# RHnejad/3D_PoseEstimation

Measured on AMD Instinct MI355X. Metric: poses/sec fwd+bwd, 17-joint lifting batch 4096; MPJPE vs ref, higher is better.
Workload: dtype f16x3 (two fp16 planes per fp32 operand, 3 fp16 MFMAs per product, fp32 accumulate); 1 GPU; BASELINE configs[1]: phase1_lifting LinearModel 34-1024-2x(1024-1024)-51, BN+ReLU+Dropout(0.5), one train_1.py step = zero_grad+forward+MSE+backward+AdamW; launch=hipgraph (one hipGraph replay per step), per_gpu_batch=4096, global_batch=4096, parallelism=dp1

## Files before the change

3d_poseestimation_amd/csrc/api.hip:

```cpp
#include <stdarg.h>
#include <stdio.h>
#include <stdlib.h>

#include <vector>

#include "adamw.h"
#include "pl_internal.h"

namespace pl {

static thread_local char g_err[512] = "";

void set_error(const char* fmt, ...) {
  va_list ap;
  va_start(ap, fmt);
  vsnprintf(g_err, sizeof(g_err), fmt, ap);
  va_end(ap);
}

namespace {

inline int64_t align_up(int64_t v, int64_t a) { return (v + a - 1) / a * a; }

int check_desc(const PLDesc* d, bool need_arenas) {
// ... 75 lines not shown

int out_splits(int M, int N, int K) {
  const int tiles = ((M + 127) / 128) * ((N + 127) / 128);
  int s = 256 / tiles;
  const int kmax = K / 128;
  if (s > kmax) s = kmax;
  return s < 1 ? 1 : s;
}

enum class Lin : uint8_t {
  Skinny, Planes, Gemm,
  PlanesMid,
  F32Mid,
};
enum class Stats : uint8_t {
  None,
  InLayer,
  Small,
  InApply,
  Finalize,
};
enum class Bwd : uint8_t {
  PlanesPair, F32Pair,
  SmallLayer, SmallLayerDw,
  InAbove,
  First,
};
struct LayerRoute {
  Lin lin;
  Stats stats;
  Bwd bwd;
  int groups;
  bool bnr_fused;
};
enum class Loss : uint8_t { SmallMse, FromSlabs, PartialOnly };

struct Ws {
  int L, G, RC;
  std::vector<size_t> z, act, bits, mean, rstd, dbpart;
  size_t stat, scale, shift, coef, ga, gb, dz, slabs, outpart, dyout, mse, total;
  size_t act_bytes, bits_bytes;
  size_t slab_floats;
  bool planes;
  int pkind;
  std::vector<size_t> actp, wp;
  std::vector<size_t> sactp;
  std::vector<char> act_f32;
  size_t dzp, amax, dzscale;
  size_t skp_out, skp_in;
  std::vector<size_t> wslab;
  std::vector<LayerRoute> layer;
  bool bn_small;
  bool small_layer;
  bool top_fused;
  bool adam_rides;
  bool small_f16;
  bool eval_small;
  bool out_narrow;
  bool out_skinny;
  Loss loss;
};

Ws plan(const PLDesc* d, int64_t B) {
  Ws w;
  w.L = 1 + 2 * d->num_stage;
  const int H = d->hidden;
  w.G = gemm_stat_groups((int)B);
  w.RC = bwd_row_chunks((int)B, H);
  size_t o = 0;
  auto take = [&](size_t bytes) {
    const size_t at = o;
    o = (size_t)align_up((int64_t)(o + bytes), 256);
    return at;
// ... 25 lines not shown
  auto need = [&](int M, int N) {
    const int s = tn_splits(M, N, (int)B);
    if (s > 1) slab = std::max(slab, (size_t)s * M * N * 4);
  };
  need(H, d->in_dim);
  need(H, H);
  need(d->out_dim, H);
  {
    const int so = out_splits((int)B, d->out_dim, H);
    if (so > 1) slab = std::max(slab, (size_t)so * B * d->out_dim * 4);
    slab = std::max(slab, (size_t)skinny_chunks((int)B) * std::max(d->in_dim, d->out_dim) * H * 4);
    slab = std::max(slab, skinny_narrow_out_part_floats((int)B, H) * 4);
    if (B <= kThinGemmMaxM && B % 128) slab = std::max(slab, thin_gemm_scratch_floats((int)B, H, H) * 4);
    if (B <= kThinGemmMaxM) slab = std::max(slab, (size_t)(H / 16 + 1) * B * 64 * 4);
  }
  w.slab_floats = slab / 4;
  w.slabs = take(slab);
  w.outpart = take((size_t)std::max(colsum_chunks((int)B), skinny_in_chunks((int)B)) * d->out_dim * 4);
  w.dyout = take((size_t)B * d->out_dim * 4);
  w.mse = take(std::max(pl_mse_scratch_bytes(B * d->out_dim), (size_t)256));
  w.dzp = w.amax = w.dzscale = 0;
  w.skp_out = take((size_t)skinny_in_chunks((int)B) * d->out_dim * H * 4);
  w.skp_in = take((size_t)skinny_in_chunks((int)B) * d->in_dim * H * 4);
  if (w.planes) {
    w.wslab.push_back(0);
    for (int l = 1; l < w.L; ++l) w.wslab.push_back(take((size_t)tn_splits(H, H, (int)B) * H * H * 4));
    for (int l = 0; l + 1 < w.L; ++l) w.actp.push_back(take(w.act_bytes));
    w.wp.push_back(0);
    for (int l = 1; l < w.L; ++l) w.wp.push_back(take((size_t)H * H * 4));
    w.dzp = take(w.act_bytes);
    w.amax = take(std::max((size_t)((H + 255) / 256) * w.RC, (size_t)(B / 64) * (H / 32)) * 2 * 4);
    w.dzscale = take((size_t)w.L * 2 * 4);
  }
  if (d->dtype == PL_F16X3 && B <= kThinGemmMaxM)
    for (int l = 0; l + 1 < w.L; ++l) w.sactp.push_back(take(w.act_bytes));
  w.total = o;

  const int world = sync_world(d);
  const bool first_ok = small_first_ok(d->in_dim), mid_ok = B * world <= 512 && small_layer_ok(2, H, H);
  w.bn_small = d->bn && !w.planes && world == 1 && B >= 2 && B <= kBnSmallRows;
  w.small_layer = w.bn_small && small_layer_ok((int)B, H, H);
  w.top_fused = w.small_layer && small_top_ok(d->out_dim);
  const bool small_head = w.top_fused && (d->num_stage > 0 || first_ok);
  w.adam_rides = small_head && H % 128 == 0;
  w.small_f16 = d->dtype == PL_F16X3 && !w.sactp.empty() && first_ok;
  w.eval_small = d->bn && B <= kThinGemmMaxM && small_layer_ok(2, H, H) && first_ok && small_top_ok(d->out_dim);
  w.out_narrow = skinny_narrow_out_supported(H, d->out_dim);
  w.out_skinny = skinny_supported(d->out_dim, H);
  const int so = w.out_narrow ? skinny_narrow_out_splits((int)B, H) : 0;
  w.loss = small_head ? Loss::SmallMse : (so && mse_from_slabs_supported(so, d->out_dim)) ? Loss::FromSlabs : Loss::PartialOnly;
  for (int l = 0; l < w.L; ++l) {
    LayerRoute r;
    if (l == 0) r.lin = skinny_supported(d->in_dim, H) ? Lin::Skinny : Lin::Gemm;
    else if (w.planes) r.lin = w.pkind == 2 && mid_ok ? Lin::PlanesMid : Lin::Planes;
    else r.lin = d->bn && d->dtype != PL_BF16 && B > kBnSmallRows && mid_ok ? Lin::F32Mid : Lin::Gemm;
    r.groups = r.lin == Lin::Skinny ? skinny_stat_groups((int)B) : w.G;
    const bool tile = w.small_layer && (l > 0 || first_ok);
    if (!d->bn) r.stats = Stats::None;
    else if (w.bn_small) r.stats = tile ? Stats::InLayer : Stats::Small;
    else r.stats = world == 1 && r.groups >= 1 && r.groups <= 4 ? Stats::InApply : Stats::Finalize;
    if (l == 0) r.bwd = tile && w.L > 1 ? Bwd::InAbove : Bwd::First;
    else if (!w.small_layer) r.bwd = w.planes ? Bwd::PlanesPair : Bwd::F32Pair;
    else r.bwd = H % 128 == 0 ? Bwd::SmallLayerDw : Bwd::SmallLayer;
    r.bnr_fused = w.planes && (l < w.L - 1 || w.out_skinny);
    w.layer.push_back(r);
  }
  return w;
}

struct BnrSlab {
  float *mine, *amax_mine, *amax0;
  int64_t floats_per_rank;
  int world;
};
BnrSlab bnr_slab(const PLDesc* d, const Ws& w, void* ws, int rc, int n_amax, bool eval_bn) {
  BnrSlab b;
  float* stat = reinterpret_cast<float*>(static_cast<char*>(ws) + w.stat);
  b.world = eval_bn ? 1 : sync_world(d);
  const int64_t sums = (int64_t)2 * rc * d->hidden;
  if (b.world == 1) {
    b.mine = stat;
    b.amax_mine = b.amax0 = w.amax ? reinterpret_cast<float*>(static_cast<char*>(ws) + w.amax) : nullptr;
    b.floats_per_rank = sums;
    return b;
  }
// ... 159 lines not shown
}

extern "C" size_t pl_workspace_bytes(const PLDesc* d, int64_t B) {
  if (check_desc(d, false) != PL_OK || B <= 0) return 0;
  return plan(d, B).total;
}

extern "C" int pl_workspace_view(const PLDesc* d, int64_t B, int which, int64_t layer, size_t* off,
                                 size_t* size) {
  PL_TRY(check_desc(d, false));
  if (B <= 0 || !off || !size) PL_FAIL(PL_EINVAL, "pl_workspace_view: bad arguments");
  const Ws w = plan(d, B);
  if (layer < 0 || layer >= w.L) PL_FAIL(PL_EINVAL, "pl_workspace_view: layer %lld out of range", (long long)layer);
  const size_t hb = (size_t)d->hidden * 4;
  switch (which) {
    case 0: *off = w.z[layer]; *size = w.act_bytes; break;
    case 1:
      if (!w.act_f32[layer])
        PL_FAIL(PL_EINVAL, "pl_workspace_view: the planes path keeps the output of hidden layer %lld as 16-bit planes only", (long long)layer);
      *off = w.act[layer]; *size = w.act_bytes; break;
    case 2: *off = w.bits[layer]; *size = w.bits_bytes; break;
    case 3: *off = w.mean[layer]; *size = hb; break;
    case 4: *off = w.rstd[layer]; *size = hb; break;
    default: PL_FAIL(PL_EINVAL, "pl_workspace_view: which=%d", which);
  }
  return PL_OK;
}

extern "C" int pl_workspace_bitmap_format(const PLDesc* d, int64_t B, int64_t layer) {
  PL_TRY(check_desc(d, false));
  if (B <= 0 || layer < 0 || layer >= 1 + 2 * (int64_t)d->num_stage) PL_FAIL(PL_EINVAL, "pl_workspace_bitmap_format: bad arguments");
  return plan(d, B).layer[layer].stats == Stats::InLayer ? 1 : 0;
}

extern "C" int pl_lifter_fwd_eval(const PLDesc* d, const float* x, float* y, int64_t B, void* ws,
                                  size_t ws_bytes, void* stream) {
  PL_TRY(check_desc(d, true));
  if (!x || !y) PL_FAIL(PL_EINVAL, "pl_lifter_fwd_eval: null x/y");
  if (B <= 0) PL_FAIL(PL_ESHAPE, "pl_lifter_fwd_eval: B=%lld", (long long)B);
  const Ws w = plan(d, B);
  PL_TRY(check_ws(w, ws, ws_bytes));
  const ParamLayout P = param_layout(d);
  hipStream_t s = (hipStream_t)stream;
  const int H = d->hidden;
  if (w.eval_small) {
    const float* a_in = x;
// ... 211 lines not shown
                                 false, f32(ws, w.outpart)));
    job(f32(ws, w.skp_out), grads + P.off[4 * w.L], skinny_in_chunks(Bi), O * H, 0, 0);
    job(f32(ws, w.outpart), grads + P.off[4 * w.L + 1], skinny_in_chunks(Bi), O, 0, 0);
    GemmArgs be = {};
    const int lt = w.L - 1;
    if (!eval_bn && w.layer[lt].bnr_fused) {
      const BnrSlab sl = bnr_slab(d, w, ws, Bi / 64, (w.pkind == 2 && lt > 0) ? (Bi / 64) * (H / 32) : 0, eval_bn);
      be.bnr_z = f32(ws, w.z[lt]); be.bnr_bits = u64(ws, w.bits[lt]);
      be.bnr_mean = f32(ws, w.mean[lt]); be.bnr_rstd = f32(ws, w.rstd[lt]); be.bnr_kscale = kscale;
      be.bnr_part_dy = sl.mine; be.bnr_part_dyz = sl.mine + (size_t)(Bi / 64) * H;
      be.bnr_amax = (w.pkind == 2 && lt > 0) ? sl.amax_mine : nullptr;
    }
    PL_TRY(launch_skinny_wide_out(dy, d->params + P.off[4 * w.L], nullptr, GA, Bi, O, H, true, nullptr, nullptr, s, &be));
  } else if (do_output) {
    PL_TRY(gemm_tn_reduced(dy, O, f32(ws, w.act[w.L - 1]), H, grads + P.off[4 * w.L], O, H, Bi, slabs, s));
    PL_TRY(launch_colsum_partial(dy, Bi, O, f32(ws, w.outpart), s));
    job(f32(ws, w.outpart), grads + P.off[4 * w.L + 1], colsum_chunks(Bi), O, 0, 0);
    GemmArgs g = {};
    g.A = dy; g.B = d->params + P.off[4 * w.L]; g.C = GA; g.M = Bi; g.N = H; g.K = O; g.lda = O; g.ldb = H; g.ldc = H;
    g.split_k = 1;
    PL_TRY(launch_gemm_f32(kNN, g, s));
  }

  for (int l = l_hi; l >= l_lo; --l) {
    const Layer ly = layer_of(d, P, grads, l);
    const LayerRoute& r = w.layer[l];
    const float* gin = (l % 2 == 1) ? GB : GA;
    const uint64_t* bits = u64(ws, w.bits[l]);
    const float* z = f32(ws, w.z[l]);
    const bool pl_layer = r.bwd == Bwd::PlanesPair;
    float* dzs = (pl_layer && w.pkind == 2) ? f32(ws, w.dzscale) + 2 * l : nullptr;
    PlaneOut dzo = {nullptr, nullptr, 1.0f, dzs, 0};
    if (pl_layer) { dzo.h = u16(ws, w.dzp); dzo.l = dzo.h + BH; dzo.kind = w.pkind; }
    auto dzbuf = [&](int layer) { return (sl && (layer & 1)) ? GB : DZ; };
    float* DZl = dzbuf(l);
    if (sl && (l < l_hi || top_fused)) {
    } else if (small) {
      PL_TRY(launch_bn_small_bwd(gin, bits, z, f32(ws, w.mean[l]), f32(ws, w.rstd[l]), ly.gamma, kscale, Bi, H, DZl, ly.ggamma,
                                 ly.gbeta, ly.gb, s, r.stats == Stats::InLayer));
    } else if (d->bn) {
      const bool fr = !eval_bn && r.bnr_fused;
      const int rc_l = fr ? Bi / 64 : w.RC;
      const int n_amax_l = fr ? (Bi / 64) * (l == w.L - 1 ? H / 32 : H / 64) : n_amax;
      const BnrSlab sl = bnr_slab(d, w, ws, rc_l, dzs ? n_amax_l : 0, eval_bn);
      float* stat = f32(ws, w.stat);
      if (!fr)
        PL_TRY(launch_bn_bwd_reduce(gin, bits, z, f32(ws, w.mean[l]), f32(ws, w.rstd[l]), kscale, Bi, H,
                                    sl.mine, sl.mine + (size_t)rc_l * H, s, 0, dzs ? sl.amax_mine : nullptr, rc_l));
      if (!eval_bn) PL_TRY(sync_gather(d, stat, sl.floats_per_rank, s));
      PL_TRY(launch_bn_bwd_finalize(stat, rc_l, eval_bn ? 1 : sync_world(d), eval_bn ? 0 : sync_rank(d), Bi, H, ly.gamma,
                                    f32(ws, w.rstd[l]), f32(ws, w.coef), ly.ggamma, ly.gbeta, s,
                                    dzs ? sl.amax0 : nullptr, n_amax_l, dzs, eval_bn ? 1 : 0, sl.floats_per_rank, sl.world));
    } else {
      PL_TRY(launch_fill(ly.ggamma, H, 0.f, s));
      PL_TRY(launch_fill(ly.gbeta, H, 0.f, s));
    }
    if (!small) {
      PL_TRY(launch_bn_bwd_dz(gin, bits, z, f32(ws, w.mean[l]), f32(ws, w.rstd[l]), f32(ws, w.coef), kscale,
                              d->bn, Bi, H, pl_layer ? nullptr : DZ, f32(ws, w.dbpart[l]), s, 0, &dzo, w.RC));
      job(f32(ws, w.dbpart[l]), ly.gb, w.RC, H, 0, 0);
    }
    const float* a_in = l == 0 ? x : (w.planes ? nullptr : f32(ws, w.act[l - 1]));
    if (pl_layer) {
      const int splits = tn_splits(H, H, Bi);
      PlanesGemmArgs nn = planes_args(w.pkind, u16(ws, w.dzp), BH, H, wplane(d, w, ws, l), (int64_t)H * H, H,
                                      (l % 2 == 1) ? GA : GB, Bi, H, H, 1.0f / kWeightPlaneScale, dzs ? dzs + 1 : nullptr);
      if (l % 2 == 1) nn.e.addend = GA;
      if (!eval_bn && w.layer[l - 1].bnr_fused) {
        const bool lower_scaled = w.pkind == 2 && l - 1 > 0;
        const BnrSlab sl = bnr_slab(d, w, ws, Bi / 64, lower_scaled ? (Bi / 64) * (H / 64) : 0, eval_bn);
        nn.e.bnr_z = f32(ws, w.z[l - 1]);
        nn.e.bnr_bits = u64(ws, w.bits[l - 1]);
        nn.e.bnr_mean = f32(ws, w.mean[l - 1]);
        nn.e.bnr_rstd = f32(ws, w.rstd[l - 1]);
        nn.e.bnr_kscale = kscale;
        nn.e.bnr_part_dy = sl.mine;
        nn.e.bnr_part_dyz = sl.mine + (size_t)(Bi / 64) * H;
        nn.e.bnr_amax = lower_scaled ? sl.amax_mine : nullptr;
      }
      float* wsl = f32(ws, w.wslab[l]);
      PlanesGemmArgs tn = planes_args(w.pkind, u16(ws, w.dzp), BH, H, u16(ws, w.actp[l - 1]), BH, H,
                                      splits > 1 ? wsl : ly.gW, H, H, Bi, 1.0f / kActPlaneScale, dzs ? dzs + 1 : nullptr);
      tn.e.split_k = splits;
      PL_TRY(launch_gemm_planes_pair(nn, tn, s));
      if (splits > 1) job(wsl, ly.gW, splits, H * H, 1, 0);
    } else if (l > 0) {
      GemmArgs g = {};
      g.A = DZl; g.B = ly.W; g.M = Bi; g.N = H; g.K = H; g.lda = H; g.ldb = H; g.ldc = H; g.split_k = 1;
      if (l % 2 == 1) { g.C = GA; g.addend = GA; } else { g.C = GB; }
      g.arith = arith_of(d);
      g.thin_scratch = slabs; g.thin_scratch_floats = w.slab_floats;
      GemmArgs t = {};
      t.arith = g.arith;
      t.A = DZl; t.B = a_in; t.M = H; t.N = H; t.K = Bi; t.lda = H; t.ldb = H; t.ldc = H; t.split_k = 1; t.C = ly.gW;
      if (sl && (r.bwd == Bwd::SmallLayer || r.bwd == Bwd::SmallLayerDw)) {
        const bool dw_rides = r.bwd == Bwd::SmallLayerDw;
        if (l - 1 >= l_lo) {
          const bool w1 = l == 1 && w.layer[0].bwd == Bwd::InAbove;
          AdamWRide ar = {};
          if (adam_rides) ar = ride(P.off[4 * l + 1], l == w.L - 1 ? P.total : P.off[4 * (l + 1) + 1]);
          PL_TRY(launch_small_layer_bwd(DZl, ly.W, (l % 2 == 1) ? GA : nullptr, (l % 2 == 1) ? GA : nullptr, Bi, H, H,
// ... 5 lines not shown
          PL_TRY(launch_gemm_f32(kNN, g, s));
        }
        PL_TRY(launch_gemm_f32(kTN, t, s));
        continue;
      }
      const int splits = tn_splits(H, H, Bi);
      t.split_k = splits; t.C = splits > 1 ? slabs : ly.gW;
      PL_TRY(launch_gemm_f32_pair(g, t, s));
      if (splits > 1) PL_TRY(launch_reduce_slabs(slabs, splits, (int64_t)H * H, ly.gW, s));
    } else if (r.bwd == Bwd::InAbove && sl && l_hi > 0) {
    } else if (r.lin == Lin::Skinny) {
      PL_TRY(launch_skinny_wide_in(a_in, DZ, ly.gW, Bi, ly.K, H, true, f32(ws, w.skp_in), s, false));
      job(f32(ws, w.skp_in), ly.gW, skinny_in_chunks(Bi), ly.K * H, 0, ly.K);
    } else {
      PL_TRY(gemm_tn_reduced(DZ, H, a_in, ly.K, ly.gW, H, ly.K, Bi, slabs, s));
    }
    if (l == 0 && dx) {
      GemmArgs g = {};
      g.A = DZ; g.B = ly.W; g.C = dx; g.M = Bi; g.N = d->in_dim; g.K = H; g.lda = H; g.ldb = d->in_dim;
      g.ldc = d->in_dim; g.split_k = 1;
      PL_TRY(launch_gemm_f32(kNN, g, s));
    }
  }
  float inv_n = 0.f;
  uint64_t* tick = nullptr;
  if (loss_out && !top_fused) {
    const int64_t n = B * O;
    job(f32(ws, w.mse), loss_out, n_loss_part, 1, 2, 0);
    inv_n = 1.0f / (float)n;
    tick = const_cast<uint64_t*>(d->step_dev);
  }
  if (!jpart.empty())
    PL_TRY(launch_reduce_rows_multi(jpart.data(), jR.data(), jH.data(), jout.data(), (int)jpart.size(), s, jkind.data(),
                                    jtrans.data(), inv_n, tick));
  if (adam) {
    const int64_t n = adam_rides ? (w.L > 1 ? P.off[4 * 1 + 1] : P.total) : P.total;
    float* p = const_cast<float*>(d->params);
    if (adam->lr_dev)
      PL_TRY(pl_adamw_flat_dev(p, grads, adam->m, adam->v, n, adam->lr_dev, adam->beta1, adam->beta2, adam->eps,
                               adam->weight_decay, adam->t, adam->t_dev, 1.0f, stream));
    else
      PL_TRY(pl_adamw_flat(p, grads, adam->m, adam->v, n, adam->lr, adam->beta1, adam->beta2, adam->eps, adam->weight_decay,
                           adam->t, 1.0f, stream));
  }
  return PL_OK;
}
// ... 334 lines not shown
```

3d_poseestimation_amd/csrc/gemm_planes.hip:

```cpp
#include "gemm_planes16.h"
#include "pl_internal.h"
#include "plane_store.h"

namespace pl {
namespace {

struct PlanesKern {
  plp::PlanesArgs p;
  GemmArgs e;
  float out_scale;
  const float* dyn_inv;
  int nt_store;
};

__device__ __forceinline__ float xadd16(const float v) {
  const auto r = __builtin_amdgcn_permlane16_swap(__float_as_uint(v), __float_as_uint(v), false, false);
  return __uint_as_float(r[0]) + __uint_as_float(r[1]);
}
__device__ __forceinline__ float xadd32(const float v) {
  const auto r = __builtin_amdgcn_permlane32_swap(__float_as_uint(v), __float_as_uint(v), false, false);
  return __uint_as_float(r[0]) + __uint_as_float(r[1]);
}
__device__ __forceinline__ float4 xadd_rows(float4 s) {
  s.x = xadd32(xadd16(s.x)); s.y = xadd32(xadd16(s.y)); s.z = xadd32(xadd16(s.z)); s.w = xadd32(xadd16(s.w));
// ... 220 lines not shown
  };
  if constexpr (WIDE) plp::planes_run16w<A_KS, B_KS, MODE, EDGE, CONV, PERSIST>(k.p, block_id, nblocks, nwork, lds, epi);
  else plp::planes_run16<A_KS, B_KS, MODE, EDGE, CONV, PERSIST, NST, T64>(k.p, block_id, nblocks, nwork, lds, epi);
}

template <bool A_KS, bool B_KS, int MODE, bool EDGE = false, int CONV = 0>
__global__ __launch_bounds__(512) void planes_gemm_kernel(PlanesKern k) {
  __shared__ __attribute__((aligned(16))) char lds[lds_bytes<MODE>()];
  planes_body<A_KS, B_KS, MODE, EDGE, CONV>(k, blockIdx.x, gridDim.x, gridDim.x, lds);
}

template <int MODE, bool EDGE, int CONV>
__global__ __launch_bounds__(512) void planes_gemm_persistent_kernel(PlanesKern k, int nwork) {
  __shared__ __attribute__((aligned(16))) char lds[lds_bytes<MODE, true>()];
  planes_body<false, false, MODE, EDGE, CONV, true>(k, blockIdx.x, gridDim.x, nwork, lds);
}

template <int MODE, bool EDGE, int CONV, bool PERSIST>
__global__ __launch_bounds__(512) void planes_gemm_t64_kernel(PlanesKern k, int nwork) {
  __shared__ __attribute__((aligned(16))) char lds[lds_bytes<MODE, PERSIST, false, true>()];
  planes_body<false, false, MODE, EDGE, CONV, PERSIST, false, true>(k, blockIdx.x, gridDim.x, nwork, lds);
}

template <int MODE, bool EDGE, int CONV, bool PERSIST>
__global__ __launch_bounds__(512) void planes_gemm_wide_kernel(PlanesKern k, int nwork) {
  __shared__ __attribute__((aligned(16))) char lds[lds_bytes<MODE, PERSIST, true>()];
  planes_body<false, false, MODE, EDGE, CONV, PERSIST, true>(k, blockIdx.x, gridDim.x, nwork, lds);
}

template <int MODE, int ER, bool EDGE>
__device__ __forceinline__ void acc_epilogue(const PlanesKern& k, plp::f32x4v (&acc)[plp::ModeCfg<MODE>::NACC][4][4], float* ldsw,
                                             const int m0, const int n0, const int slice, const int wm, const int wn, const int lane) {
  const float os = MODE == plp::kF16x3 ? (k.dyn_inv ? k.out_scale * k.dyn_inv[0] : k.out_scale) : 1.f;
  const int q = lane >> 4, c = lane & 15, lc = c * 4;
  float4 v[16];
#pragma unroll
  for (int pass = 0; pass < 64 / ER; ++pass) {
#pragma unroll
    for (int r2 = 0; r2 < ER / 16; ++r2)
#pragma unroll
      for (int ct = 0; ct < 4; ++ct)
#pragma unroll
        for (int r = 0; r < 4; ++r) {
          float x = acc[0][pass * (ER / 16) + r2][ct][r];
          if constexpr (MODE == plp::kF16x3) x = fmaf(acc[1][pass * (ER / 16) + r2][ct][r], 1.0f / plp::kF16LoScale, x) * os;
          ldsw[(r2 * 16 + 4 * q + r) * 68 + ct * 16 + c] = x;
        }
#pragma unroll
    for (int it = 0; it < ER / 4; ++it)
      v[pass * (ER / 4) + it] = *reinterpret_cast<const float4*>(ldsw + (it * 4 + q) * 68 + lc);
  }
  float* C = k.e.C ? k.e.C + (k.e.split_k > 1 ? (size_t)slice * k.e.M * k.e.ldc : 0) : nullptr;
  staged_epilogue<EDGE>(k, C, v, m0, n0, wm, wn, lane);
}

template <int MODE>
__global__ __launch_bounds__(512) void planes_gemm_chain_kernel(PlanesKern k0, PlanesKern k1) {
  __shared__ __attribute__((aligned(16))) char lds[ring_bytes<MODE>() + stage_bytes<32>()];
  const int lane = threadIdx.x & 63, wave = threadIdx.x >> 6;
  const int wm = (wave & 3) >> 1, wn = wave & 1;
  float* ldsw = reinterpret_cast<float*>(lds + ring_bytes<MODE>()) + (wave & 3) * 32 * 68;
  auto epi0 = [&](plp::f32x4v (&acc)[plp::ModeCfg<MODE>::NACC][4][4], const int m0, const int n0, const int slice) {
    acc_epilogue<MODE, 32, false>(k0, acc, ldsw, m0, n0, slice, wm, wn, lane);
  };
  auto epi1 = [&](plp::f32x4v (&acc)[plp::ModeCfg<MODE>::NACC][4][4], const int m0, const int n0, const int slice) {
    acc_epilogue<MODE, 32, false>(k1, acc, ldsw, m0, n0, slice, wm, wn, lane);
  };
  plp::planes_run16_chain<MODE>(k0.p, k1.p, blockIdx.x, gridDim.x, lds, epi0, epi1);
}

template <int MODE>
__global__ __launch_bounds__(512) void planes_gemm_dual_kernel(PlanesKern k0, PlanesKern k1, int n0) {
  __shared__ __attribute__((aligned(16))) char lds[lds_bytes<MODE>()];
  const int b = blockIdx.x;
  if (b < n0)
    planes_body<false, true, MODE>(k0, b, n0, n0, lds);
  else
    planes_body<true, true, MODE>(k1, b - n0, gridDim.x - n0, gridDim.x - n0, lds);
}

PlanesKern kern_of(GemmLayout layout, const PlanesGemmArgs& a) {
  PlanesKern k = {};
  k.p.A = reinterpret_cast<const __bf16*>(a.A);
  k.p.B = reinterpret_cast<const __bf16*>(a.B);
  k.p.C = a.e.C;
  k.p.M = a.e.M; k.p.N = a.e.N; k.p.K = a.e.K;
  k.p.lda = a.lda; k.p.ldb = a.ldb; k.p.ldc = a.e.ldc;
  k.p.split_k = a.e.split_k;
  k.p.a_plane = (size_t)a.a_plane; k.p.b_plane = (size_t)a.b_plane;
  k.e = a.e;
  k.p.cv_cin = a.e.conv_cin; k.p.cv_h = a.e.conv_h; k.p.cv_w = a.e.conv_w; k.p.cv_ho = a.e.conv_ho; k.p.cv_wo = a.e.conv_wo;
  k.p.cv_kw = a.e.conv_kw; k.p.cv_stride = a.e.conv_stride; k.p.cv_pad_h = a.e.conv_pad_h; k.p.cv_pad_w = a.e.conv_pad_w;
  k.p.cv_stride_w = a.e.conv_stride_w > 0 ? a.e.conv_stride_w : a.e.conv_stride;
  k.out_scale = a.out_scale;
  k.dyn_inv = a.dyn_inv;
  k.nt_store = (int64_t)a.e.M * a.e.N * 4 >= kNontemporalBytes ? 1 : 0;
  (void)layout;
  return k;
}

int cu_count() {
// ... 59 lines not shown
                       reinterpret_cast<uintptr_t>(e.stat_m2) | reinterpret_cast<uintptr_t>(e.bnr_z) |
                       reinterpret_cast<uintptr_t>(e.bnr_mean) | reinterpret_cast<uintptr_t>(e.bnr_rstd) |
                       reinterpret_cast<uintptr_t>(e.bnr_part_dy) | reinterpret_cast<uintptr_t>(e.bnr_part_dyz);
  if (al & 15) return false;
  return true;
}

int launch_gemm_planes(GemmLayout layout, const PlanesGemmArgs& a, hipStream_t s) {
  if (!planes_gemm_ok(layout, a)) PL_FAIL(PL_ESHAPE, "gemm_planes: unsupported problem %dx%dx%d (layout %d, mode %d)", a.e.M, a.e.N, a.e.K, (int)layout, a.mode);
  const PlanesKern k = kern_of(layout, a);
  const dim3 grid(grid_of(a)), block(512);
  void* prof = prof_begin_flops(2.0 * a.e.M * a.e.N * a.e.K, s);
#define PL_PLANES_LAUNCH(MODE, EDGE)                                                                             \
  switch (layout) {                                                                                              \
    case kNT: hipLaunchKernelGGL((planes_gemm_kernel<false, false, MODE, EDGE>), grid, block, 0, s, k); break;   \
    case kNN: hipLaunchKernelGGL((planes_gemm_kernel<false, true, MODE, EDGE>), grid, block, 0, s, k); break;    \
    case kTN: hipLaunchKernelGGL((planes_gemm_kernel<true, true, MODE, EDGE>), grid, block, 0, s, k); break;     \
    default: PL_FAIL(PL_EINVAL, "gemm_planes: bad layout %d", (int)layout);                                     \
  }
  const int ncu = cu_count();
  const bool persist = layout == kNT && (int)grid.x >= 2 * ncu;
  const bool wide = layout == kNT && splits_of(a.e) == 1 && a.e.K % 64 == 0 && a.e.K >= 1024 &&
                    (a.e.conv_cin == 0 || a.e.conv_cin % 64 == 0);
  const bool t64 = layout == kNT && a.e.N <= 64 && splits_of(a.e) == 1 && !a.e.scat_on;
  if (t64) {
    const int nwork = (int)(((a.e.M + 255) / 256) * ((a.e.N + 63) / 64));
    const bool pers = nwork >= 2 * ncu;
    const dim3 tg(pers ? ncu : nwork);
    const bool edge = (a.e.M % 256) != 0 || (a.e.N % 64) != 0 || a.e.conv_cin;
#define PL_T64(MODE, P)                                                                                                  \
    if (a.e.conv_cin) hipLaunchKernelGGL((planes_gemm_t64_kernel<MODE, true, 1, P>), tg, block, 0, s, k, nwork);          \
    else if (edge) hipLaunchKernelGGL((planes_gemm_t64_kernel<MODE, true, 0, P>), tg, block, 0, s, k, nwork);             \
    else hipLaunchKernelGGL((planes_gemm_t64_kernel<MODE, false, 0, P>), tg, block, 0, s, k, nwork);
    if (pers) { if (a.mode == plp::kF16x3) { PL_T64(plp::kF16x3, true) } else { PL_T64(plp::kBf16, true) } }
    else { if (a.mode == plp::kF16x3) { PL_T64(plp::kF16x3, false) } else { PL_T64(plp::kBf16, false) } }
#undef PL_T64
  } else if (wide) {
    const int nwork = (int)grid.x;
    const dim3 wg(persist ? ncu : nwork);
    const bool edge = is_edge(a) || a.e.conv_cin;
#define PL_WIDE(MODE, P)                                                                                                  \
    if (a.e.conv_cin) hipLaunchKernelGGL((planes_gemm_wide_kernel<MODE, true, 1, P>), wg, block, 0, s, k, nwork);          \
    else if (edge) hipLaunchKernelGGL((planes_gemm_wide_kernel<MODE, true, 0, P>), wg, block, 0, s, k, nwork);             \
    else hipLaunchKernelGGL((planes_gemm_wide_kernel<MODE, false, 0, P>), wg, block, 0, s, k, nwork);
    if (persist) { if (a.mode == plp::kF16x3) { PL_WIDE(plp::kF16x3, true) } else { PL_WIDE(plp::kBf16, true) } }
    else { if (a.mode == plp::kF16x3) { PL_WIDE(plp::kF16x3, false) } else { PL_WIDE(plp::kBf16, false) } }
#undef PL_WIDE
  } else if (persist) {
// ... 28 lines not shown
int launch_gemm_planes_pair(const PlanesGemmArgs& nn, const PlanesGemmArgs& tn, hipStream_t s) {
  if (!planes_gemm_ok(kNN, nn) || !planes_gemm_ok(kTN, tn) || nn.mode != tn.mode || is_edge(nn) || is_edge(tn))
    PL_FAIL(PL_ESHAPE, "gemm_planes_pair: unsupported problems");
  const PlanesKern k0 = kern_of(kNN, nn), k1 = kern_of(kTN, tn);
  const int g0 = grid_of(nn), g1 = grid_of(tn);
  void* prof = prof_begin_flops(2.0 * nn.e.M * nn.e.N * nn.e.K + 2.0 * tn.e.M * tn.e.N * tn.e.K, s);
  if (g0 == g1 && nn.e.K % 32 == 0 && nn.e.K >= 64 && tn.e.K % (32 * splits_of(tn.e)) == 0 &&
      tn.e.K >= 32 * splits_of(tn.e)) {
    const dim3 cg(g0), cb(512);
    if (nn.mode == plp::kF16x3) hipLaunchKernelGGL((planes_gemm_chain_kernel<plp::kF16x3>), cg, cb, 0, s, k0, k1);
    else hipLaunchKernelGGL((planes_gemm_chain_kernel<plp::kBf16>), cg, cb, 0, s, k0, k1);
    prof_end(prof, s);
    PL_CHECK_LAUNCH("gemm_planes_chain");
    return PL_OK;
  }
  const dim3 grid(g0 + g1), block(512);
  if (nn.mode == plp::kF16x3) hipLaunchKernelGGL((planes_gemm_dual_kernel<plp::kF16x3>), grid, block, 0, s, k0, k1, g0);
  else hipLaunchKernelGGL((planes_gemm_dual_kernel<plp::kBf16>), grid, block, 0, s, k0, k1, g0);
  prof_end(prof, s);
  PL_CHECK_LAUNCH("gemm_planes_dual");
  return PL_OK;
}

}
```

3d_poseestimation_amd/csrc/gemm_planes16.h:

```cpp
#pragma once
#include "gemm_planes.h"

namespace plp {

typedef float f32x4v __attribute__((ext_vector_type(4)));

__device__ __forceinline__ int kc16_swz(int row) { return (0 - (row >> 2)) & 3; }

template <bool KS>
__device__ __forceinline__ uint32_t glds_lane_off16(int rb, int lane, int ld, int left = 0x7fffffff) {
  if (!KS) {
    const int row = rb * 16 + (lane >> 2);
    const int ch = (lane & 3) ^ kc16_swz(row);
    return (uint32_t)(min(row, left - 1) * ld * 2 + ch * 16);
  }
  const int krow = rb * 4 + (lane >> 4);
  const int ch = (lane & 15) ^ ((((lane >> 4) & 3) << 2) | (rb & 3));
  return (uint32_t)(krow * ld * 2 + min(ch, (left >> 3) - 1) * 16);
}

template <bool KS>
struct FragAddr16 {
  uint32_t b[KS ? 8 : 1];
  __device__ __forceinline__ void init(int wq, int lane) {
// ... 13 lines not shown
          b[t * 2 + u] = (uint32_t)(256 * row + 16 * (ch ^ x) + 8 * (pp & 1));
        }
    }
  }
};

template <bool KS>
__device__ __forceinline__ s16x8 read_frag16(const char* op, const FragAddr16<KS>& fa, int t) {
  if (!KS) return *reinterpret_cast<const s16x8*>(op + fa.b[0] + t * 1024);
  const s16x4 lo = __builtin_amdgcn_ds_read_tr16_b64_v4i16((__attribute__((address_space(3))) s16x4*)(op + fa.b[t * 2 + 0]));
  const s16x4 hi = __builtin_amdgcn_ds_read_tr16_b64_v4i16((__attribute__((address_space(3))) s16x4*)(op + fa.b[t * 2 + 1]));
  return __builtin_shufflevector(lo, hi, 0, 1, 2, 3, 4, 5, 6, 7);
}

template <int MODE>
__device__ __forceinline__ f32x4v mfma16x16(const s16x8 a, const s16x8 b, const f32x4v c) {
  if constexpr (MODE == kF16x3)
    return __builtin_amdgcn_mfma_f32_16x16x32_f16(__builtin_bit_cast(f16x8, a), __builtin_bit_cast(f16x8, b), c, 0, 0, 0);
  else
    return __builtin_amdgcn_mfma_f32_16x16x32_bf16(__builtin_bit_cast(bf16x8, a), __builtin_bit_cast(bf16x8, b), c, 0, 0, 0);
}

constexpr int kDmaOutOfRange = 0x7ffffff0;
template <bool A_KS, bool B_KS, int MODE, bool EDGE, int CONV, bool PERSIST, int NST, bool T64, class Epi>
__device__ __forceinline__ void planes_run16(const PlanesArgs& p, const int block_id, const int nblocks, const int nwork,
                                             char* __restrict__ lds, Epi&& epi) {
  static_assert(MODE == kF16x3 || MODE == kBf16, "two fp16 planes or one bf16 plane");
  constexpr int NPL = ModeCfg<MODE>::NPL, NACC = ModeCfg<MODE>::NACC;
  static_assert(!T64 || (!A_KS && !B_KS), "the 256 x 64 tile is an NT tile");
  constexpr int TM = T64 ? 256 : 128, TNW = T64 ? 64 : 128;
  constexpr int OPPA = (A_KS ? 128 : TM) * 64, OPPB = (B_KS ? 128 : TNW) * 64;
  constexpr int STAGE = NPL * (OPPA + OPPB);
  constexpr int JA = OPPA / 4096, JB = OPPB / 4096;
  constexpr int NDMA = NPL * (JA + JB);
  static_assert(NST >= 3 && (NST - 2) * NDMA <= 63, "ring depth: vmcnt counts at most 63 requests");
  const int tid = threadIdx.x;
  const int lane = tid & 63;
  const int wave = __builtin_amdgcn_readfirstlane(tid >> 6);
  const bool loader = wave >= 4;
  const int lw = wave & 3;
  const int wm = T64 ? (wave & 3) : (wave & 3) >> 1, wn = T64 ? 0 : (wave & 1);

  const int tiles_n = EDGE ? (p.N + TNW - 1) / TNW : p.N / TNW;
  const int splits = p.split_k > 1 ? p.split_k : 1;
  const int ntiles = nwork / splits;
  int item_lo, item_hi;
  if (PERSIST) {
    const int per = (nwork + nblocks - 1) / nblocks;
    item_lo = min(block_id * per, nwork);
    item_hi = min(item_lo + per, nwork);
  } else {
    item_lo = block_id;
    if ((nwork & 7) == 0) item_lo = (block_id & 7) * (nwork >> 3) + (block_id >> 3);
    item_hi = item_lo + 1;
  }
  if (item_lo >= item_hi) return;
  const int per_slice = ((p.K / 32 + splits - 1) / splits) * 32;
  auto decode = [&](const int w, int& m0, int& n0, int& slice, int& kbeg) {
    slice = w / ntiles;
    const int t = w - slice * ntiles;
    m0 = (t / tiles_n) * TM;
    n0 = (t % tiles_n) * TNW;
    kbeg = 0;
    int kend = p.K;
    if (splits > 1) {
      kbeg = min(slice * per_slice, p.K);
      kend = min(kbeg + per_slice, p.K);
    }
    return (kend - kbeg) / 32;
  };

  const int ga_step = A_KS ? 32 * p.lda * 2 : 64;
  const int gb_step = B_KS ? 32 * p.ldb * 2 : 64;
  auto barrier = [&]() {
    __builtin_amdgcn_sched_barrier(0);
    __builtin_amdgcn_s_barrier();
    __builtin_amdgcn_sched_barrier(0);
  };
  auto next_stage = [](const int o) { return o + STAGE == NST * STAGE ? 0 : o + STAGE; };
  int st[2] = {0, STAGE};
  auto rotate = [&]() { st[0] = st[1]; st[1] = next_stage(st[1]); };

  if (loader) {
// ... 756 lines not shown
```

3d_poseestimation_amd/csrc/pl_internal.h:

```cpp
#pragma once
#include <hip/hip_runtime.h>
#include <stddef.h>
#include <stdint.h>

#include "../../include/poselift.h"

namespace pl {

constexpr int kWave = 64;

void set_error(const char* fmt, ...);

#define PL_FAIL(code, ...)        \
  do {                            \
    ::pl::set_error(__VA_ARGS__); \
    return (code);                \
  } while (0)

#define PL_CHECK_LAUNCH(what)                                              \
  do {                                                                     \
    hipError_t e__ = hipGetLastError();                                    \
    if (e__ != hipSuccess)                                                 \
      PL_FAIL(PL_EHIP, "%s: launch failed: %s", what, hipGetErrorString(e__)); \
  } while (0)
// ... 56 lines not shown
uint32_t* range_record();
inline int range_site_act(int layer) { return PL_RANGE_SITE_LIFTER_ACT + (layer < 7 ? layer : 7); }
inline void range_watch(PlaneOut& po, int site) {
  if (po.kind == 2 && !po.dyn) { po.range = range_record(); po.site = site; }
}
constexpr long long kNontemporalBytes = 64ll << 20;
constexpr float kActPlaneScale = 1.0f;
constexpr float kWeightPlaneScale = 16.0f;
constexpr float kConvActPlaneScale = 1.0f / 64.0f;

struct PlanesGemmArgs {
  GemmArgs e;
  const unsigned short* A;
  const unsigned short* B;
  int64_t a_plane, b_plane;
  int lda, ldb;
  int mode;
  float out_scale;
  const float* dyn_inv;
};
bool planes_gemm_ok(GemmLayout layout, const PlanesGemmArgs& a);
int launch_gemm_planes(GemmLayout layout, const PlanesGemmArgs& a, hipStream_t s);
int launch_gemm_planes_pair(const PlanesGemmArgs& nn, const PlanesGemmArgs& tn, hipStream_t s);
int launch_split_planes(const float* x, int64_t n, const PlaneOut& out, hipStream_t s);
int plane_out_of(int mode, void* planes, int64_t n, float scale, const float* dyn, PlaneOut* po, const char* who);

int launch_gemm_f32(GemmLayout layout, const GemmArgs& a, hipStream_t s);
constexpr int kThinGemmMaxM = 512;
bool thin_gemm_ok(GemmLayout layout, const GemmArgs& a);
size_t thin_gemm_scratch_floats(int M, int N, int K);
int launch_gemm_thin(GemmLayout layout, const GemmArgs& a, float* scratch, size_t scratch_floats, hipStream_t s);
int launch_gemm_f32_pair(const GemmArgs& nn, const GemmArgs& tn, hipStream_t s);
int gemm_stat_groups(int M);
int prof_enable(int on);
void* prof_begin_flops(double flops, hipStream_t s);
void prof_end(void* rec, hipStream_t s);
int prof_read(double min_flops, double max_flops, double* ms_total, int64_t* launches, double* flops_total);

inline int bitmap_words_per_row(int H) { return ((H + 255) / 256) * 4; }

int launch_bn_finalize(const float* stat, int G, int world, int B, int H,
                       const float* gamma, const float* beta, float eps, float momentum,
                       float* running_mean, float* running_var, int64_t* batches,
                       float* mean, float* rstd, float* scale, float* shift, hipStream_t s, int group_rows = 64);

struct BnFinalizeArgs {
// ... 108 lines not shown
```

Baseline: 6.665 million poses/s.

## Defer hidden-layer weight-gradient GEMMs into one batched TN launch after backward

In the planes backward path, each hidden layer now keeps its dz planes in a per-layer slab and launches only the dX (NN) GEMM. All weight-gradient (TN) products are then issued together in a single batched kernel at the end. This replaces the per-layer NN+TN pair launches and gives the dW products a larger grid that can fill the GPU. The split-K slices are accumulated in place, with the slices of a tile run in order within a block. A wide NN kernel variant with K-strided B is also routed in for large K. The cost is extra workspace per layer for the dz planes, and the dW work no longer overlaps the per-layer dX kernels.

```diff
diff --git a/3d_poseestimation_amd/csrc/api.hip b/3d_poseestimation_amd/csrc/api.hip
--- a/3d_poseestimation_amd/csrc/api.hip
+++ b/3d_poseestimation_amd/csrc/api.hip
@@ -121,6 +121,7 @@
 };
 enum class Bwd : uint8_t {
   PlanesPair, F32Pair,
+  PlanesDeferred,
   SmallLayer, SmallLayerDw,
   InAbove,
   First,
@@ -148,6 +149,7 @@
   size_t dzp, amax, dzscale;
   size_t skp_out, skp_in;
   std::vector<size_t> wslab;
+  bool dw_deferred;
   std::vector<LayerRoute> layer;
   bool bn_small;
   bool small_layer;
@@ -219,9 +221,11 @@
   w.dzp = w.amax = w.dzscale = 0;
   w.skp_out = take((size_t)skinny_in_chunks((int)B) * d->out_dim * H * 4);
   w.skp_in = take((size_t)skinny_in_chunks((int)B) * d->in_dim * H * 4);
+  w.dw_deferred = w.planes && w.L - 1 <= kMaxTnBatch && (int64_t)(w.L - 1) * (H / 128) * (H / 128) == (B / 128) * (H / 128);
   if (w.planes) {
+    const size_t per_layer = std::max((size_t)tn_splits(H, H, (int)B) * H * H * 4, w.dw_deferred ? w.act_bytes : (size_t)0);
     w.wslab.push_back(0);
-    for (int l = 1; l < w.L; ++l) w.wslab.push_back(take((size_t)tn_splits(H, H, (int)B) * H * H * 4));
+    for (int l = 1; l < w.L; ++l) w.wslab.push_back(take(per_layer));
     for (int l = 0; l + 1 < w.L; ++l) w.actp.push_back(take(w.act_bytes));
     w.wp.push_back(0);
     for (int l = 1; l < w.L; ++l) w.wp.push_back(take((size_t)H * H * 4));
@@ -257,7 +261,7 @@
     else if (w.bn_small) r.stats = tile ? Stats::InLayer : Stats::Small;
     else r.stats = world == 1 && r.groups >= 1 && r.groups <= 4 ? Stats::InApply : Stats::Finalize;
     if (l == 0) r.bwd = tile && w.L > 1 ? Bwd::InAbove : Bwd::First;
-    else if (!w.small_layer) r.bwd = w.planes ? Bwd::PlanesPair : Bwd::F32Pair;
+    else if (!w.small_layer) r.bwd = w.dw_deferred ? Bwd::PlanesDeferred : w.planes ? Bwd::PlanesPair : Bwd::F32Pair;
     else r.bwd = H % 128 == 0 ? Bwd::SmallLayerDw : Bwd::SmallLayer;
     r.bnr_fused = w.planes && (l < w.L - 1 || w.out_skinny);
     w.layer.push_back(r);
@@ -463,6 +467,10 @@
     case 2: *off = w.bits[layer]; *size = w.bits_bytes; break;
     case 3: *off = w.mean[layer]; *size = hb; break;
     case 4: *off = w.rstd[layer]; *size = hb; break;
+    case 5:
+      if (!w.planes || layer < 1)
+        PL_FAIL(PL_EINVAL, "pl_workspace_view: hidden layer %lld has no dz planes", (long long)layer);
+      *off = w.dw_deferred ? w.wslab[layer] : w.dzp; *size = w.act_bytes; break;
     default: PL_FAIL(PL_EINVAL, "pl_workspace_view: which=%d", which);
   }
   return PL_OK;
@@ -720,16 +728,19 @@
     PL_TRY(launch_gemm_f32(kNN, g, s));
   }
 
+  const bool dw_deferred = w.dw_deferred && !eval_bn && l_hi == w.L - 1 && l_lo == 0;
+  PlanesTnBatch dwt = {};
+  dwt.n = w.L - 1;
   for (int l = l_hi; l >= l_lo; --l) {
     const Layer ly = layer_of(d, P, grads, l);
     const LayerRoute& r = w.layer[l];
     const float* gin = (l % 2 == 1) ? GB : GA;
     const uint64_t* bits = u64(ws, w.bits[l]);
     const float* z = f32(ws, w.z[l]);
-    const bool pl_layer = r.bwd == Bwd::PlanesPair;
+    const bool pl_layer = r.bwd == Bwd::PlanesPair || r.bwd == Bwd::PlanesDeferred;
     float* dzs = (pl_layer && w.pkind == 2) ? f32(ws, w.dzscale) + 2 * l : nullptr;
     PlaneOut dzo = {nullptr, nullptr, 1.0f, dzs, 0};
-    if (pl_layer) { dzo.h = u16(ws, w.dzp); dzo.l = dzo.h + BH; dzo.kind = w.pkind; }
+    if (pl_layer) { dzo.h = u16(ws, dw_deferred ? w.wslab[l] : w.dzp); dzo.l = dzo.h + BH; dzo.kind = w.pkind; }
     auto dzbuf = [&](int layer) { return (sl && (layer & 1)) ? GB : DZ; };
     float* DZl = dzbuf(l);
     if (sl && (l < l_hi || top_fused)) {
@@ -761,7 +772,7 @@
     const float* a_in = l == 0 ? x : (w.planes ? nullptr : f32(ws, w.act[l - 1]));
     if (pl_layer) {
       const int splits = tn_splits(H, H, Bi);
-      PlanesGemmArgs nn = planes_args(w.pkind, u16(ws, w.dzp), BH, H, wplane(d, w, ws, l), (int64_t)H * H, H,
+      PlanesGemmArgs nn = planes_args(w.pkind, dzo.h, BH, H, wplane(d, w, ws, l), (int64_t)H * H, H,
                                       (l % 2 == 1) ? GA : GB, Bi, H, H, 1.0f / kWeightPlaneScale, dzs ? dzs + 1 : nullptr);
       if (l % 2 == 1) nn.e.addend = GA;
       if (!eval_bn && w.layer[l - 1].bnr_fused) {
@@ -775,6 +786,11 @@
         nn.e.bnr_part_dy = sl.mine;
         nn.e.bnr_part_dyz = sl.mine + (size_t)(Bi / 64) * H;
         nn.e.bnr_amax = lower_scaled ? sl.amax_mine : nullptr;
+      }
+      if (dw_deferred) {
+        PL_TRY(launch_gemm_planes(kNN, nn, s));
+        dwt.A[l - 1] = dzo.h; dwt.B[l - 1] = u16(ws, w.actp[l - 1]); dwt.C[l - 1] = ly.gW; dwt.dyn_inv[l - 1] = dzs ? dzs + 1 : nullptr;
+        continue;
       }
       float* wsl = f32(ws, w.wslab[l]);
       PlanesGemmArgs tn = planes_args(w.pkind, u16(ws, w.dzp), BH, H, u16(ws, w.actp[l - 1]), BH, H,
@@ -826,6 +842,11 @@
       PL_TRY(launch_gemm_f32(kNN, g, s));
     }
   }
+  if (dw_deferred) {
+    PlanesGemmArgs tn = planes_args(w.pkind, dwt.A[0], BH, H, dwt.B[0], BH, H, dwt.C[0], H, H, Bi, 1.0f / kActPlaneScale, dwt.dyn_inv[0]);
+    tn.e.split_k = tn_splits(H, H, Bi);
+    PL_TRY(launch_gemm_planes_tn_batch(tn, dwt, s));
+  }
   float inv_n = 0.f;
   uint64_t* tick = nullptr;
   if (loss_out && !top_fused) {
diff --git a/3d_poseestimation_amd/csrc/gemm_planes.hip b/3d_poseestimation_amd/csrc/gemm_planes.hip
--- a/3d_poseestimation_amd/csrc/gemm_planes.hip
+++ b/3d_poseestimation_amd/csrc/gemm_planes.hip
@@ -266,18 +266,17 @@
   planes_body<false, false, MODE, EDGE, CONV, PERSIST, false, true>(k, blockIdx.x, gridDim.x, nwork, lds);
 }
 
-template <int MODE, bool EDGE, int CONV, bool PERSIST>
+template <int MODE, bool EDGE, int CONV, bool PERSIST, bool B_KS = false>
 __global__ __launch_bounds__(512) void planes_gemm_wide_kernel(PlanesKern k, int nwork) {
   __shared__ __attribute__((aligned(16))) char lds[lds_bytes<MODE, PERSIST, true>()];
-  planes_body<false, false, MODE, EDGE, CONV, PERSIST, true>(k, blockIdx.x, gridDim.x, nwork, lds);
-}
-
-template <int MODE, int ER, bool EDGE>
-__device__ __forceinline__ void acc_epilogue(const PlanesKern& k, plp::f32x4v (&acc)[plp::ModeCfg<MODE>::NACC][4][4], float* ldsw,
-                                             const int m0, const int n0, const int slice, const int wm, const int wn, const int lane) {
+  planes_body<false, B_KS, MODE, EDGE, CONV, PERSIST, true>(k, blockIdx.x, gridDim.x, nwork, lds);
+}
+
+template <int MODE, int ER>
+__device__ __forceinline__ void acc_rows(const PlanesKern& k, plp::f32x4v (&acc)[plp::ModeCfg<MODE>::NACC][4][4], float* ldsw,
+                                         const int lane, float4 (&v)[16]) {
   const float os = MODE == plp::kF16x3 ? (k.dyn_inv ? k.out_scale * k.dyn_inv[0] : k.out_scale) : 1.f;
   const int q = lane >> 4, c = lane & 15, lc = c * 4;
-  float4 v[16];
 #pragma unroll
   for (int pass = 0; pass < 64 / ER; ++pass) {
 #pragma unroll
@@ -294,6 +293,12 @@
     for (int it = 0; it < ER / 4; ++it)
       v[pass * (ER / 4) + it] = *reinterpret_cast<const float4*>(ldsw + (it * 4 + q) * 68 + lc);
   }
+}
+template <int MODE, int ER, bool EDGE>
+__device__ __forceinline__ void acc_epilogue(const PlanesKern& k, plp::f32x4v (&acc)[plp::ModeCfg<MODE>::NACC][4][4], float* ldsw,
+                                             const int m0, const int n0, const int slice, const int wm, const int wn, const int lane) {
+  float4 v[16];
+  acc_rows<MODE, ER>(k, acc, ldsw, lane, v);
   float* C = k.e.C ? k.e.C + (k.e.split_k > 1 ? (size_t)slice * k.e.M * k.e.ldc : 0) : nullptr;
   staged_epilogue<EDGE>(k, C, v, m0, n0, wm, wn, lane);
 }
@@ -321,6 +326,45 @@
     planes_body<false, true, MODE>(k0, b, n0, n0, lds);
   else
     planes_body<true, true, MODE>(k1, b - n0, gridDim.x - n0, gridDim.x - n0, lds);
+}
+
+struct TnBatchTab {
+  const __bf16* A[kMaxTnBatch];
+  const __bf16* B[kMaxTnBatch];
+  float* C[kMaxTnBatch];
+  const float* dyn_inv[kMaxTnBatch];
+};
+template <int MODE>
+__global__ __launch_bounds__(512) void planes_gemm_tn_batch_kernel(PlanesKern k, TnBatchTab t, int tiles) {
+  __shared__ __attribute__((aligned(16))) char lds[lds_bytes<MODE, true>()];
+  const int i = __builtin_amdgcn_readfirstlane((int)blockIdx.x / tiles);
+  int b = (int)blockIdx.x - i * tiles;
+  if ((tiles & 7) == 0) b = (b & 7) * (tiles >> 3) + (b >> 3);
+  PlanesKern ki = k;
+  ki.p.A = t.A[i];
+  ki.p.B = t.B[i];
+  ki.p.C = ki.e.C = t.C[i];
+  ki.dyn_inv = t.dyn_inv[i];
+  const int lane = threadIdx.x & 63, wave = threadIdx.x >> 6;
+  const int wm = (wave & 3) >> 1, wn = wave & 1;
+  constexpr int NST = persist_nst<MODE>();
+  float* ldsw = reinterpret_cast<float*>(lds + ring_bytes<MODE, NST>()) + (wave & 3) * kPersistRows * 68;
+  const int splits = k.p.split_k > 1 ? k.p.split_k : 1;
+  auto epi = [&](plp::f32x4v (&acc)[plp::ModeCfg<MODE>::NACC][4][4], const int m0, const int n0, const int slice) {
+    float4 v[16];
+    acc_rows<MODE, kPersistRows>(ki, acc, ldsw, lane, v);
+    float* c0 = ki.e.C + (size_t)(m0 + wm * 64 + (lane >> 4)) * ki.e.ldc + n0 + wn * 64 + (lane & 15) * 4;
+    if (slice > 0) {
+      float4 q[16];
+#pragma unroll
+      for (int it = 0; it < 16; ++it) q[it] = *reinterpret_cast<const float4*>(c0 + (size_t)it * 4 * ki.e.ldc);
+#pragma unroll
+      for (int it = 0; it < 16; ++it) { v[it].x = q[it].x + v[it].x; v[it].y = q[it].y + v[it].y; v[it].z = q[it].z + v[it].z; v[it].w = q[it].w + v[it].w; }
+    }
+#pragma unroll
+    for (int it = 0; it < 16; ++it) *reinterpret_cast<float4*>(c0 + (size_t)it * 4 * ki.e.ldc) = v[it];
+  };
+  plp::planes_run16<true, true, MODE, false, 0, true, NST, false, true>(ki.p, b, tiles, tiles * splits, lds, epi);
 }
 
 PlanesKern kern_of(GemmLayout layout, const PlanesGemmArgs& a) {
@@ -426,8 +470,13 @@
   const bool persist = layout == kNT && (int)grid.x >= 2 * ncu;
   const bool wide = layout == kNT && splits_of(a.e) == 1 && a.e.K % 64 == 0 && a.e.K >= 1024 &&
                     (a.e.conv_cin == 0 || a.e.conv_cin % 64 == 0);
+  const bool wide_nn = layout == kNN && splits_of(a.e) == 1 && a.e.K % 64 == 0 && a.e.K >= 1024 && !a.e.conv_cin && !is_edge(a);
   const bool t64 = layout == kNT && a.e.N <= 64 && splits_of(a.e) == 1 && !a.e.scat_on;
-  if (t64) {
+  if (wide_nn) {
+    const int nwork = (int)grid.x;
+    if (a.mode == plp::kF16x3) hipLaunchKernelGGL((planes_gemm_wide_kernel<plp::kF16x3, false, 0, false, true>), grid, block, 0, s, k, nwork);
+    else hipLaunchKernelGGL((planes_gemm_wide_kernel<plp::kBf16, false, 0, false, true>), grid, block, 0, s, k, nwork);
+  } else if (t64) {
     const int nwork = (int)(((a.e.M + 255) / 256) * ((a.e.N + 63) / 64));
     const bool pers = nwork >= 2 * ncu;
     const dim3 tg(pers ? ncu : nwork);
@@ -502,4 +551,33 @@
   return PL_OK;
 }
 
-}
+int launch_gemm_planes_tn_batch(const PlanesGemmArgs& shape, const PlanesTnBatch& t, hipStream_t s) {
+  if (t.n < 1 || t.n > kMaxTnBatch) PL_FAIL(PL_EINVAL, "gemm_planes_tn_batch: %d problems (1 .. %d)", t.n, kMaxTnBatch);
+  const GemmArgs& e = shape.e;
+  if (e.bias || e.addend || e.resid || e.col_scale || e.stat_sum || e.bnr_z || e.cpl_kind || e.conv_cin)
+    PL_FAIL(PL_EINVAL, "gemm_planes_tn_batch: plain products only");
+  TnBatchTab tab = {};
+  for (int i = 0; i < t.n; ++i) {
+    PlanesGemmArgs a = shape;
+    a.A = t.A[i]; a.B = t.B[i]; a.e.C = t.C[i]; a.dyn_inv = t.dyn_inv[i];
+    if (!planes_gemm_ok(kTN, a) || is_edge(a))
+      PL_FAIL(PL_ESHAPE, "gemm_planes_tn_batch: unsupported problem %d (%dx%dx%d, mode %d)", i, e.M, e.N, e.K, shape.mode);
+    tab.A[i] = reinterpret_cast<const __bf16*>(t.A[i]);
+    tab.B[i] = reinterpret_cast<const __bf16*>(t.B[i]);
+    tab.C[i] = t.C[i];
+    tab.dyn_inv[i] = shape.mode == plp::kF16x3 ? t.dyn_inv[i] : nullptr;
+  }
+  PlanesGemmArgs a0 = shape;
+  a0.A = t.A[0]; a0.B = t.B[0]; a0.e.C = t.C[0]; a0.dyn_inv = t.dyn_inv[0];
+  const PlanesKern k = kern_of(kTN, a0);
+  const int tiles = grid_of(a0) / splits_of(e);
+  const dim3 grid(tiles * t.n), block(512);
+  void* prof = prof_begin_flops(2.0 * e.M * e.N * e.K * t.n, s);
+  if (shape.mode == plp::kF16x3) hipLaunchKernelGGL((planes_gemm_tn_batch_kernel<plp::kF16x3>), grid, block, 0, s, k, tab, tiles);
+  else hipLaunchKernelGGL((planes_gemm_tn_batch_kernel<plp::kBf16>), grid, block, 0, s, k, tab, tiles);
+  prof_end(prof, s);
+  PL_CHECK_LAUNCH("gemm_planes_tn_batch");
+  return PL_OK;
+}
+
+}
diff --git a/3d_poseestimation_amd/csrc/gemm_planes16.h b/3d_poseestimation_amd/csrc/gemm_planes16.h
--- a/3d_poseestimation_amd/csrc/gemm_planes16.h
+++ b/3d_poseestimation_amd/csrc/gemm_planes16.h
@@ -59,7 +59,7 @@
 }
 
 constexpr int kDmaOutOfRange = 0x7ffffff0;
-template <bool A_KS, bool B_KS, int MODE, bool EDGE, int CONV, bool PERSIST, int NST, bool T64, class Epi>
+template <bool A_KS, bool B_KS, int MODE, bool EDGE, int CONV, bool PERSIST, int NST, bool T64, bool TILE_MAJOR = false, class Epi>
 __device__ __forceinline__ void planes_run16(const PlanesArgs& p, const int block_id, const int nblocks, const int nwork,
                                              char* __restrict__ lds, Epi&& epi) {
   static_assert(MODE == kF16x3 || MODE == kBf16, "two fp16 planes or one bf16 plane");
@@ -94,8 +94,9 @@
   if (item_lo >= item_hi) return;
   const int per_slice = ((p.K / 32 + splits - 1) / splits) * 32;
   auto decode = [&](const int w, int& m0, int& n0, int& slice, int& kbeg) {
-    slice = w / ntiles;
-    const int t = w - slice * ntiles;
+    int t;
+    if (TILE_MAJOR) { t = w / splits; slice = w - t * splits; }
+    else { slice = w / ntiles; t = w - slice * ntiles; }
     m0 = (t / tiles_n) * TM;
     n0 = (t % tiles_n) * TNW;
     kbeg = 0;
diff --git a/3d_poseestimation_amd/csrc/pl_internal.h b/3d_poseestimation_amd/csrc/pl_internal.h
--- a/3d_poseestimation_amd/csrc/pl_internal.h
+++ b/3d_poseestimation_amd/csrc/pl_internal.h
@@ -102,6 +102,15 @@
 bool planes_gemm_ok(GemmLayout layout, const PlanesGemmArgs& a);
 int launch_gemm_planes(GemmLayout layout, const PlanesGemmArgs& a, hipStream_t s);
 int launch_gemm_planes_pair(const PlanesGemmArgs& nn, const PlanesGemmArgs& tn, hipStream_t s);
+constexpr int kMaxTnBatch = 8;
+struct PlanesTnBatch {
+  int n;
+  const unsigned short* A[kMaxTnBatch];
+  const unsigned short* B[kMaxTnBatch];
+  float* C[kMaxTnBatch];
+  const float* dyn_inv[kMaxTnBatch];
+};
+int launch_gemm_planes_tn_batch(const PlanesGemmArgs& shape, const PlanesTnBatch& t, hipStream_t s);
 int launch_split_planes(const float* x, int64_t n, const PlaneOut& out, hipStream_t s);
 int plane_out_of(int mode, void* planes, int64_t n, float scale, const float* dyn, PlaneOut* po, const char* who);
 
```

Result: no change. 6.713 million poses/s (median of 2 runs) (+0.7%).
